# conix-center/pointcloud_stitching

Measured on AMD Instinct MI355X. Metric: Mpoints/s stitched (8x1280x720 streams: deproject+transform+RGB+pack), higher is better.
Workload: dtype f32

## Files before the change

### pointcloud_stitching_amd/csrc/pcs_capi.cpp

```cpp

#include <algorithm>
#include <cmath>
#include <cstdarg>
#include <cstdio>
#include <cstdlib>
#include <cstring>
#include <exception>
#include <new>
#include <string>
#include <vector>

#include "pcs_host.h"

using namespace pcs_host;

namespace pcs_host {

thread_local std::string g_create_err;

int fail(pcs_ctx* c, int status, const char* fmt, ...)
{
    char buf[512];
    va_list ap;
    va_start(ap, fmt);
// ... 946 lines not shown
}

int pcs_process_frames_device_batch(pcs_ctx* c, int n_sets, const uint16_t* const* d_depth, const uint8_t* const* d_color,
                                    int16_t* const* d_payload, size_t payload_shorts, int32_t* const* d_counts)
try {
    if (!c) return PCS_ERR_INVALID_ARG;
    if (n_sets < 0) return fail(c, PCS_ERR_INVALID_ARG, "n_sets %d < 0", n_sets);
    if (n_sets == 0) return PCS_OK;
    if (!d_depth || !d_color || !d_payload) return fail(c, PCS_ERR_INVALID_ARG, "NULL pointer");
    const int S = c->n_streams;
    bool aligned = true;
    for (int k = 0; k < n_sets; k++) {
        if (!d_payload[k]) return fail(c, PCS_ERR_INVALID_ARG, "frame-set %d: NULL payload pointer", k);
        if ((uintptr_t)d_payload[k] & 1u) return fail(c, PCS_ERR_INVALID_ARG, "frame-set %d: payload pointer must be 2-byte aligned", k);
        aligned &= ((uintptr_t)d_payload[k] & 15u) == 0;
        for (int s = 0; s < S; s++) {
            if (!d_depth[(size_t)k * S + s] || !d_color[(size_t)k * S + s])
                return fail(c, PCS_ERR_INVALID_ARG, "frame-set %d stream %d: NULL raster pointer", k, s);
            if ((uintptr_t)d_depth[(size_t)k * S + s] & 1u)
                return fail(c, PCS_ERR_INVALID_ARG, "frame-set %d stream %d: depth pointer not 2-byte aligned", k, s);
        }
    }
    DeviceGuard guard(c->device);
    const int per_launch = std::min(kBatchSets, kBatchEntries / S);
    const bool dense = !has_pred(c->flags) && c->downsample == 1 && c->dense_ok && aligned && per_launch >= 2;
    if (has_pred(c->flags) && c->downsample == 1 && per_launch >= 2 && S <= kLaunchStreams) {
        if (payload_shorts < c->max_payload_points * PCS_POINT_SHORTS)
            return fail(c, PCS_ERR_CAPACITY, "payload buffers hold %zu shorts; with compaction the worst case %zu is required",
                        payload_shorts, c->max_payload_points * PCS_POINT_SHORTS);
        const size_t tt = std::max<uint32_t>(c->total_tiles, 1);
        const size_t row = 2 * tt + (size_t)S + (size_t)(S + 1);
        if (c->batch_scratch_sets < per_launch) {
            if (c->d_batch_scratch) { HIPCHK(c, hipStreamSynchronize(c->stream)); (void)hipFree(c->d_batch_scratch); c->d_batch_scratch = nullptr; }
            c->batch_scratch_sets = 0;
            HIPCHK(c, hipMalloc((void**)&c->d_batch_scratch, sizeof(uint32_t) * row * per_launch));
            c->batch_scratch_sets = per_launch;
        }
        uint32_t* tcounts = c->d_batch_scratch;
        uint32_t* tprefix = tcounts + tt * per_launch;
        uint32_t* kept    = tprefix + tt * per_launch;
        int32_t*  icounts = reinterpret_cast<int32_t*>(kept + (size_t)S * per_launch);
        bool fast = true, ident = true;
        for (int s = 0; s < S; s++) { fast &= c->h_params[s].cert_fast != 0; ident &= c->h_params[s].ident_r != 0; }
        const MathSel sel = !fast ? MathSel::Ieee : (ident ? MathSel::CertIdentR : MathSel::Cert);
        std::pair<hipEvent_t, hipEvent_t> ev{};
        if (c->kernel_timing) {
            int rc = acquire_event_pair(c, ev);
            if (rc) return rc;
            HIPCHK(c, hipEventRecord(ev.first, c->stream));
        }
        for (int k0 = 0; k0 < n_sets; k0 += per_launch) {
            const int nk = std::min(per_launch, n_sets - k0);
            BatchPtrs bp{};
            BatchCounts bc{};
            for (int k = 0; k < nk; k++) {
                bp.payload[k] = reinterpret_cast<uint8_t*>(d_payload[k0 + k]);
                bc.counts[k] = (d_counts && d_counts[k0 + k]) ? d_counts[k0 + k] : icounts + (size_t)k * (S + 1);
                for (int s = 0; s < S; s++) {
                    bp.depth[k * S + s] = d_depth[(size_t)(k0 + k) * S + s];
                    bp.color[k * S + s] = d_color[(size_t)(k0 + k) * S + s];
                }
            }
            HIPCHK(c, launch_compact_batch(c->d_params, S, nk, c->max_points, c->total_tiles, c->flags, sel, bp, bc,
                                           tcounts, tprefix, kept, c->stream));
        }
        if (c->kernel_timing) {
            HIPCHK(c, hipEventRecord(ev.second, c->stream));
            c->ev_pool.push_back(ev);
        }
        return PCS_OK;
    }
    if (!dense) {
        for (int k = 0; k < n_sets; k++) {
            int rc = run_fused_device(c, d_depth + (size_t)k * S, d_color + (size_t)k * S, d_payload[k], payload_shorts,
                                      d_counts ? d_counts[k] : nullptr);
            if (rc) return rc;
        }
        return PCS_OK;
    }
    if (payload_shorts < c->max_payload_points * PCS_POINT_SHORTS)
        return fail(c, PCS_ERR_CAPACITY, "payload buffers hold %zu shorts, %zu needed", payload_shorts,
                    c->max_payload_points * PCS_POINT_SHORTS);
    bool fast = true, ident = true, noovf = true, dd = false, cd = false;
    for (int s = 0; s < S; s++) {
        const StreamParams& q = c->h_params[s];
        fast &= q.cert_fast != 0; ident &= q.ident_r != 0; noovf &= q.no_overflow != 0;
        dd |= q.ddist != 0;
        cd |= q.cdist != 0 || q.tex_half != 0;
    }
    const MathSel sel = !fast ? MathSel::Ieee
                      : noovf ? (ident ? MathSel::CertIdentRNoOvf : MathSel::CertNoOvf)
                              : (ident ? MathSel::CertIdentR : MathSel::Cert);
    std::pair<hipEvent_t, hipEvent_t> ev{};
    if (c->kernel_timing) {
        int rc = acquire_event_pair(c, ev);
        if (rc) return rc;
        HIPCHK(c, hipEventRecord(ev.first, c->stream));
    }
    for (int k0 = 0; k0 < n_sets; k0 += per_launch) {
        const int nk = std::min(per_launch, n_sets - k0);
        BatchPtrs bp{};
        for (int k = 0; k < nk; k++) {
            bp.payload[k] = reinterpret_cast<uint8_t*>(d_payload[k0 + k]);
            for (int s = 0; s < S; s++) {
                bp.depth[k * S + s] = d_depth[(size_t)(k0 + k) * S + s];
                bp.color[k * S + s] = d_color[(size_t)(k0 + k) * S + s];
            }
        }
        HIPCHK(c, launch_fused_dense_batch(c->d_params, S, nk, c->max_points, dd, cd, sel, bp, c->stream));
    }
    if (d_counts)
        for (int k = 0; k < n_sets; k++)
            if (d_counts[k])
                HIPCHK(c, hipMemcpyAsync(d_counts[k], c->d_static_counts, sizeof(int32_t) * (S + 1), hipMemcpyDeviceToDevice, c->stream));
    if (c->kernel_timing) {
        HIPCHK(c, hipEventRecord(ev.second, c->stream));
        c->ev_pool.push_back(ev);
    }
    return PCS_OK;
} catch (const std::exception& ex) {
    return fail(c, PCS_ERR_NOMEM, "pcs_process_frames_device_batch: host allocation failed (%s)", ex.what());
}

int pcs_process_frames(pcs_ctx* c, const uint16_t* const* depth, const uint8_t* const* color, int16_t* stitched,
                       size_t stitched_shorts, int write_header, int* points_per_stream, int* out_size_bytes)
try {
    if (!c) return PCS_ERR_INVALID_ARG;
    if (!depth || !color || !stitched) return fail(c, PCS_ERR_INVALID_ARG, "NULL pointer");
    DeviceGuard guard(c->device);
    int rc;
    for (int s = 0; s < c->n_streams; s++)
        if (!depth[s] || !color[s]) return fail(c, PCS_ERR_INVALID_ARG, "stream %d: NULL raster pointer", s);
    {
        const size_t need = PCS_HEADER_SHORTS + c->max_payload_points * PCS_POINT_SHORTS;
        std::vector<const uint16_t*> zd(c->n_streams);
        std::vector<const uint8_t*> zcol(c->n_streams);
        void* zout = nullptr;
        bool zero_copy = zero_copy_enabled() && stitched_shorts >= need && ((uintptr_t)stitched & 3u) == 0;
        for (int s = 0; s < c->n_streams; s++) {
            void *a = nullptr, *b = nullptr;
            const int va = host_device_view(c, depth[s], (size_t)c->h_params[s].n_points * sizeof(uint16_t), &a);
            const int vb = host_device_view(c, color[s], c->h_params[s].color_bytes, &b);
            if (va < 0 || vb < 0) return partly_locked(c, va < 0 ? "depth raster" : "colour raster", s);
            zero_copy = zero_copy && va == 1 && vb == 1;
            zd[s] = static_cast<const uint16_t*>(a); zcol[s] = static_cast<const uint8_t*>(b);
        }
        {
            const int vo = host_device_view(c, stitched, std::min(stitched_shorts, need) * sizeof(int16_t), &zout);
            if (vo < 0) return partly_locked(c, "stitched buffer", 0);
            zero_copy = zero_copy && vo == 1;
        }
        if (zero_copy) {
            int16_t* zpay = static_cast<int16_t*>(zout) + PCS_HEADER_SHORTS;
            rc = run_fused_device(c, zd.data(), zcol.data(), zpay, c->max_payload_points * PCS_POINT_SHORTS, c->d_counts, true);
            if (rc) return rc;
            std::vector<int32_t> h(c->n_streams + 1);
            HIPCHK(c, hipMemcpyAsync(h.data(), c->d_counts, h.size() * sizeof(int32_t), hipMemcpyDeviceToHost, c->stream));
            HIPCHK(c, hipStreamSynchronize(c->stream));
            const int32_t size = (int32_t)((size_t)h[c->n_streams] * PCS_POINT_BYTES);
            if (write_header) std::memcpy(stitched, &size, sizeof size);
            if (points_per_stream) for (int s = 0; s < c->n_streams; s++) points_per_stream[s] = h[s];
            if (out_size_bytes) *out_size_bytes = size;
            return PCS_OK;
        }
    }
    if ((rc = ensure_rasters(c))) return rc;
    for (int s = 0; s < c->n_streams; s++) {
        const StreamParams& P = c->h_params[s];
        const size_t db = (size_t)P.n_points * sizeof(uint16_t);
        HIPCHK(c, hipMemcpyAsync(c->s_depth[s], depth[s], db, hipMemcpyHostToDevice, c->stream));
        HIPCHK(c, hipMemcpyAsync(c->s_color[s], color[s], P.color_bytes, hipMemcpyHostToDevice, c->stream));
    }
    const size_t max_bytes = c->max_payload_points * PCS_POINT_BYTES;
    if ((rc = ensure(c, c->s_payload, c->s_payload_cap, max_bytes + 16))) return rc;
    rc = run_fused_device(c, c->s_depth.data(), c->s_color.data(), c->s_payload, c->max_payload_points * PCS_POINT_SHORTS,
// ... 436 lines not shown
```

### pointcloud_stitching_amd/csrc/pcs_kernels.hip

```cpp

#include "pcs_kernels_common.h"

#ifndef EMIT_WAVES
#define EMIT_WAVES 6
#endif

namespace pcs {

namespace {

constexpr uint32_t kDenseStageBytes = kTilePoints * PCS_POINT_BYTES;
constexpr uint32_t kStageBytes      = kTilePoints * PCS_POINT_BYTES + 32;

__device__ __forceinline__ void stage_record(uint8_t* lds, uint32_t off, const Record& r)
{
    const bool odd = (off & 2u) != 0u;
    const uint32_t yz = perm(r.zc, r.xy, kHiLo);
    const uint32_t cc = perm(r.b, r.zc, kHiLo);
    const uint32_t h_val = odd ? r.xy : r.b;
    const uint32_t a_val = odd ? yz : r.xy;
    const uint32_t b_val = odd ? cc : r.zc;
    const uint32_t h_off = odd ? off : off + 8u;
    const uint32_t a_off = odd ? off + 2u : off;
    *reinterpret_cast<uint16_t*>(lds + h_off) = (uint16_t)h_val;
// ... 74 lines not shown
__device__ __forceinline__ void dense_tile(const StreamParams& P, const Src& src, const uint8_t* __restrict__ color,
                                           uint32_t tile0, uint32_t n, uint8_t* __restrict__ out_bytes,
                                           uint4* stage)
{
    const uint32_t i0 = tile0 + threadIdx.x * kPointsPerLane;
    PointIn p[8];
    src.load8(P, i0, n, p);

    uint32_t w[20];
    auto fill = [&](auto& cv) {
#pragma unroll
        for (int k = 0; k < 8; k += 2) {
            const Record a = make_record(P, color, p[k], cv);
            const Record b = make_record(P, color, p[k + 1], cv);
            uint32_t* o = w + (k >> 1) * 5;
            o[0] = a.xy;
            o[1] = a.zc;
            o[2] = perm(b.xy, a.b, kLoLo);
            o[3] = perm(b.zc, b.xy, kHiLo);
            o[4] = perm(b.b, b.zc, kHiLo);
        }
    };
    if (Src::Math::kCvtMode == 2) {
        FastCvt<false> fast;
        fill(fast);
        if (__builtin_expect(fast.redo(), 0)) { ExactCvt exact; fill(exact); }
    } else if (Src::Math::kCvtMode == 1) {
        FastCvt<true> fast;
        fill(fast);
        if (__builtin_expect(fast.redo(), 0)) { ExactCvt exact; fill(exact); }
    } else {
        ExactCvt exact;
        fill(exact);
    }
    uint4* mine = stage + threadIdx.x * 5;
#pragma unroll
    for (int k = 0; k < 5; k++) mine[k] = make_uint4(w[4 * k], w[4 * k + 1], w[4 * k + 2], w[4 * k + 3]);
    __syncthreads();

    const uint32_t pts = min(THREADS * kPointsPerLane, n - tile0);
    store_staged<THREADS>(reinterpret_cast<const uint8_t*>(stage), 0u, pts * PCS_POINT_BYTES,
                          out_bytes + (size_t)tile0 * PCS_POINT_BYTES);
}

constexpr uint32_t kWaveStageBytes = 64u * kPointsPerLane * PCS_POINT_BYTES;
constexpr uint32_t kWinPieces      = 3;
constexpr uint32_t kWinBytes       = kWinPieces * 64u * 16u;
constexpr uint32_t kWinZeroWord    = kWaveStageBytes - 16u;
static_assert(kWinBytes + 8u <= kWinZeroWord, "the windows, the dword read past their end and the zero word fit one wave's stage");

template <class T> using cptr = const __attribute__((address_space(4))) T*;

__device__ __forceinline__ void color_stretch(const StreamParams& P, const int32_t (&wp)[3], int32_t crow, int32_t c0, int32_t c1,
                                              uint32_t room, uint32_t& ws, uint32_t& len)
{
    const int32_t lo = min(max((c0 * wp[0] + wp[1]) >> 12, 0), P.cW - 1);
    const int32_t hi = min(max((c1 * wp[0] + wp[2]) >> 12, 0), P.cW - 1);
    const uint32_t row = (uint32_t)crow * (uint32_t)P.stride;
    ws = (row + (uint32_t)lo * (uint32_t)P.bpp) & ~15u;
    const uint32_t we = min((row + (uint32_t)hi * (uint32_t)P.bpp + 4u + 15u) & ~15u, P.color_bytes & ~15u);
    len = min(we > ws ? we - ws : 0u, room);
}

typedef uint32_t u32x4v __attribute__((ext_vector_type(4)));
__device__ __forceinline__ u32x4v load16_asm(const void* base, uint32_t off)
{
    u32x4v v;
    asm volatile("global_load_dwordx4 %0, %1, %2" : "=v"(v) : "v"(off), "s"(base));
    return v;
}
__device__ __forceinline__ uint32_t load4_asm(const void* base, uint32_t off)
{
    uint32_t v;
    asm volatile("global_load_dword %0, %1, %2" : "=v"(v) : "v"(off), "s"(base));
    return v;
}
__device__ __forceinline__ void window_piece(const uint8_t* color, uint32_t off, uint32_t lds)
{
    uint32_t keep;
    asm volatile("s_mov_b32 %0, m0\n\ts_mov_b32 m0, %3\n\ts_nop 0\n\tglobal_load_lds_dwordx4 %1, %2\n\ts_mov_b32 m0, %0"
                 : "=&s"(keep) : "v"(off), "s"(color), "s"(lds) : "memory");
}

template <class Mth, uint32_t THREADS = kBlockThreads>
__device__ __forceinline__ void dense_tile_rowc(const StreamParams& P, const uint16_t* __restrict__ depth,
                                                const uint8_t* __restrict__ color, uint32_t tile0, uint32_t n,
                                                uint8_t* __restrict__ out_bytes, uint4* stage)
{
    static_assert(Mth::kRowConst && Mth::kCvtMode == 2, "the no-overflow row-constant policy");
    const uint32_t i0 = tile0 + threadIdx.x * kPointsPerLane;
    const uint32_t ic = min(i0, n - kPointsPerLane);
    const uint32_t r = P.w_magic ? (__umulhi(ic, P.w_magic) >> P.w_shift) : ic / (uint32_t)P.W;
    const uint32_t c0 = ic - r * (uint32_t)P.W;
    u32x4v dv = load16_asm(depth, ic * 2u);
    u32x4v ma = load16_asm(P.mx, c0 * 4u);
    u32x4v mb = load16_asm(P.mx, c0 * 4u + 16u);
    uint32_t myb = load4_asm(P.my, r * 4u);
    uint32_t crow = load4_asm(P.my, ((uint32_t)P.H + r) * 4u);

    const uint32_t wave = __builtin_amdgcn_readfirstlane(threadIdx.x >> 6);
    const uint32_t iw = tile0 + wave * 64u * kPointsPerLane;
    const uint32_t il = min(iw + 64u * kPointsPerLane, n) - 1u;
    const uint32_t ra = __builtin_amdgcn_readfirstlane(r), rb = __builtin_amdgcn_readlane(r, 63);
    const cptr<int32_t> tab = (cptr<int32_t>)(uintptr_t)(P.my + P.H);
    const int32_t wp[3] = {tab[P.H], tab[P.H + 1], tab[P.H + 2]};
    const uint32_t lrel = wave * kWaveStageBytes;
    uint32_t wsa = 0, lena = 0, wsb = 0, lenb = 0;
    if (iw < n) {
        color_stretch(P, wp, tab[ra], (int32_t)(iw - ra * (uint32_t)P.W), ra == rb ? (int32_t)(il - ra * (uint32_t)P.W) : P.W - 1,
                      kWinBytes, wsa, lena);
        if (rb != ra) color_stretch(P, wp, tab[rb], 0, (int32_t)(il - rb * (uint32_t)P.W), kWinBytes - lena, wsb, lenb);
    }
    const uint32_t lane = threadIdx.x & 63u;
    const uint32_t pieces = max((lena + lenb) >> 4, 1u), pa = lena >> 4;
    const uint32_t lds0 = (uint32_t)(uintptr_t)(__attribute__((address_space(3))) uint8_t*)stage + lrel;
#pragma unroll
    for (uint32_t k = 0; k < kWinPieces; k++) {
        const uint32_t j = min(k * 64u + lane, pieces - 1u);
        window_piece(color, j < pa ? wsa + 16u * j : wsb + 16u * (j - pa), lds0 + k * 1024u);
    }
    if (lane == 0) *reinterpret_cast<uint32_t*>(reinterpret_cast<uint8_t*>(stage) + lrel + kWinZeroWord) = *(cptr<uint32_t>)(uintptr_t)color;

    static_assert(kWinPieces == 3, "the wait below leaves the window's requests in flight");
    asm volatile("s_waitcnt vmcnt(3)" : "+v"(dv), "+v"(ma), "+v"(mb), "+v"(myb), "+v"(crow));
    PointIn p[8];
    {
        const uint32_t dw[4] = {dv.x, dv.y, dv.z, dv.w};
        const uint32_t mxs[8] = {ma.x, ma.y, ma.z, ma.w, mb.x, mb.y, mb.z, mb.w};
#pragma unroll
        for (int k = 0; k < 8; k++) {
            const uint32_t d = (k & 1) ? (dw[k >> 1] >> 16) : (dw[k >> 1] & 0xFFFFu);
            p[k] = deproject_pixel_rowc<Mth>(P, d, __uint_as_float(mxs[k]), __uint_as_float(myb), (int)crow);
        }
    }
    FastCvt<false> cv;
    uint32_t xy[8], zz[8], ci[8];
#pragma unroll
    for (int k = 0; k < 8; k++) {
        const float ax = world_mm(P.M + 0, p[k].X, p[k].Y, p[k].Z);
        const float ay = world_mm(P.M + 4, p[k].X, p[k].Y, p[k].Z);
        const float az = world_mm(P.M + 8, p[k].X, p[k].Y, p[k].Z);
        xy[k] = perm((uint32_t)cv.cvt(ay), (uint32_t)cv.cvt(ax), kLoLo);
        zz[k] = (uint32_t)cv.cvt(az);
        const int32_t xi = cv.pixel(__fmaf_rn(p[k].u, P.c_w_f, 0.5f), P.cW - 1, P.c_wm1_f);
        ci[k] = __umul24((uint32_t)xi, (uint32_t)P.bpp) + __umul24((uint32_t)__float_as_int(p[k].v), (uint32_t)P.stride);
    }
    const bool in_a = r == ra;
    const uint32_t ws = in_a ? wsa : wsb, len = in_a ? lena : lenb;
    const uint32_t wn = len > 3u ? len - 3u : 0u;
    const uint32_t lb = lrel + (in_a ? 0u : lena), lz = lrel + kWinZeroWord;
    asm volatile("s_waitcnt vmcnt(0)" : "+v"(ci[0]), "+v"(ci[1]), "+v"(ci[2]), "+v"(ci[3]), "+v"(ci[4]), "+v"(ci[5]), "+v"(ci[6]),
                 "+v"(ci[7]) :: "memory");
    uint32_t wc[8];
    bool miss = false;
#pragma unroll
    for (int k = 0; k < 8; k++) {
        const uint32_t o = ci[k] - ws;
        const bool in = o < wn;
        const uint32_t* qa = reinterpret_cast<const uint32_t*>(reinterpret_cast<const uint8_t*>(stage) + (in ? (lb + o) & ~3u : lz));
        wc[k] = __builtin_amdgcn_alignbyte(qa[1], qa[0], ci[k]);
        miss |= !in && ci[k] != 0u;
    }
    if (__builtin_expect(miss, 0)) {
#pragma unroll
        for (int k = 0; k < 8; k++) {
            if (!(ci[k] - ws < wn) && ci[k] != 0u) {
                ExactCvt exact;
                uint32_t shift;
                const uint32_t off = exact.window(ci[k], P.color_bytes - 4u, shift);
                uint32_t g;
                __builtin_memcpy(&g, color + off, 4);
                wc[k] = g >> shift;
            }
        }
    }
    uint32_t w[20];
#pragma unroll
    for (int k = 0; k < 8; k += 2) {
        const Record a{xy[k], perm(wc[k], zz[k], kLoLo), __builtin_amdgcn_ubfe(wc[k], 16, 8)};
        const Record b{xy[k + 1], perm(wc[k + 1], zz[k + 1], kLoLo), __builtin_amdgcn_ubfe(wc[k + 1], 16, 8)};
        uint32_t* o = w + (k >> 1) * 5;
        o[0] = a.xy;
        o[1] = a.zc;
        o[2] = perm(b.xy, a.b, kLoLo);
        o[3] = perm(b.zc, b.xy, kHiLo);
        o[4] = perm(b.b, b.zc, kHiLo);
    }
    uint4* mine = stage + threadIdx.x * 5;
#pragma unroll
    for (int k = 0; k < 5; k++) mine[k] = make_uint4(w[4 * k], w[4 * k + 1], w[4 * k + 2], w[4 * k + 3]);
    __syncthreads();

    const uint32_t pts = min(THREADS * kPointsPerLane, n - tile0);
    store_staged<THREADS>(reinterpret_cast<const uint8_t*>(stage), 0u, pts * PCS_POINT_BYTES,
                          out_bytes + (size_t)tile0 * PCS_POINT_BYTES);
}

template <class Src, bool PRED, bool DS1>
__device__ __forceinline__ void generic_tile(const StreamParams& P, const Src& src, const uint8_t* __restrict__ color,
                                             uint32_t tile0, uint32_t n, uint32_t flags, uint32_t ds,
                                             uint32_t g0, uint32_t out_first, uint8_t* __restrict__ payload_bytes,
                                             uint8_t* stage, uint32_t* wsum)
{
    if (DS1) ds = 1u;
    const uint32_t i0 = tile0 + threadIdx.x * kPointsPerLane;
    PointIn p[8];
    src.load8(P, i0, n, p);

    uint32_t keep, ex = 0;
    if (PRED) {
        keep = keep_mask8(p, i0, n, flags);
        uint32_t wave_total;
        ex = wave_exclusive_scan(__popc(keep), wave_total);
        if ((threadIdx.x & 63) == 63) wsum[threadIdx.x >> 6] = wave_total;
    } else {
        const uint32_t mine = (i0 < n) ? min(8u, n - i0) : 0u;
        keep = (1u << mine) - 1u;
    }

    Record rec[8];
    auto fill = [&](auto& cv) {
#pragma unroll
        for (int k = 0; k < 8; k++) rec[k] = make_record(P, color, p[k], cv);
    };
    if (Src::Math::kCvtMode == 2) {
        FastCvt<false> fast;
        fill(fast);
        if (__builtin_expect(fast.redo(), 0)) { ExactCvt exact; fill(exact); }
// ... 137 lines not shown
        if (__builtin_expect(fast.redo(), 0)) { ExactCvt exact; fill(exact); }
    } else if (Mth::kCvtMode == 1) {
        FastCvt<true> fast;
        fill(fast);
        if (__builtin_expect(fast.redo(), 0)) { ExactCvt exact; fill(exact); }
    } else {
        ExactCvt exact;
        fill(exact);
    }

    uint32_t own = 0, tot = 0;
    const uint32_t first = gtile - t;
    for (uint32_t j = first + threadIdx.x; j < gtile; j += kBlockThreads) own += desc_wait(a.desc + j, a.gen, a.error);
    if ((int)threadIdx.x < s) tot = desc_wait(a.stream_desc + stream0 + threadIdx.x, a.gen, a.error);
    const uint32_t tot_lane = tot;
    own = wave_sum(own);
    tot = wave_sum(tot);
    if (lane == 0) { psum[wave] = own; psum[4 + wave] = tot; }
    __syncthreads();
    const uint32_t own_excl = psum[0] + psum[1] + psum[2] + psum[3];
    const uint32_t chain = a.chain_in ? *a.chain_in : 0u;
    const uint32_t q_lo = chain + psum[4] + psum[5] + psum[6] + psum[7] + own_excl;
    if (threadIdx.x == 0 && t == tiles_s - 1) {
        __hip_atomic_store(a.stream_desc + stream0 + s, desc_pack(a.gen, kDescReady, own_excl + tile_kept), __ATOMIC_RELAXED,
                           __HIP_MEMORY_SCOPE_AGENT);
        a.stream_end[stream0 + s] = q_lo + tile_kept;
    }
    if (a.counts && s == n_launch - 1 && t == tiles_s - 1) {
        if ((int)threadIdx.x < s) a.counts[stream0 + threadIdx.x] = (int32_t)tot_lane;
        if (threadIdx.x == 0) {
            a.counts[stream0 + s] = (int32_t)(own_excl + tile_kept);
            if (a.last_launch) a.counts[a.n_total] = (int32_t)(q_lo + tile_kept);
        }
    }

    uint8_t* gdst = payload_bytes + (size_t)q_lo * PCS_POINT_BYTES;
    const uint32_t head = (uint32_t)((uintptr_t)gdst & 15u);
    uint32_t rank = lane_first;
#pragma unroll
    for (int k = 0; k < 8; k++) {
        if ((keep >> k) & 1u) {
            stage_record(stage, head + rank * PCS_POINT_BYTES, rec[k]);
            rank++;
        }
    }
    __syncthreads();
    store_staged(stage, head, tile_kept * PCS_POINT_BYTES, gdst);
}



template <bool DDIST, bool CDIST, class Mth, uint32_t THREADS = kBlockThreads>
__global__ __launch_bounds__(THREADS, 7)
void pcs_fused_dense_kernel(const StreamParams* __restrict__ params, int stream0, FramePtrs fp,
                            uint8_t* __restrict__ payload_bytes)
{
    __shared__ uint4 stage[THREADS * kPointsPerLane * PCS_POINT_BYTES / 16];
    const int s = blockIdx.y;
    const StreamParams& P = params[stream0 + s];
    request_constants(P, fp.depth[s], fp.color[s], payload_bytes);
    const uint32_t n = P.n_points;
    const uint32_t tile0 = blockIdx.x * (THREADS * kPointsPerLane);
    if (tile0 >= n) return;
    if constexpr (Mth::kRowConst) {
        dense_tile_rowc<Mth, THREADS>(P, fp.depth[s], fp.color[s], tile0, n, payload_bytes + (size_t)P.out_base * PCS_POINT_BYTES, stage);
    } else {
        DepthSource<DDIST, CDIST, Mth> src{fp.depth[s]};
        dense_tile<DepthSource<DDIST, CDIST, Mth>, THREADS>(P, src, fp.color[s], tile0, n, payload_bytes + (size_t)P.out_base * PCS_POINT_BYTES, stage);
    }
}

template <bool DDIST, bool CDIST, class Mth>
__global__ __launch_bounds__(kBlockThreads, 7)
void pcs_fused_dense_batch_kernel(const StreamParams* __restrict__ params, BatchPtrs bp)
{
    __shared__ uint4 stage[kDenseStageBytes / 16];
    const int s = blockIdx.y;
    const StreamParams& P = params[s];
    const int e = blockIdx.z * gridDim.y + s;
    request_constants(P, bp.depth[e], bp.color[e], bp.payload[blockIdx.z]);
    const uint32_t n = P.n_points;
    const uint32_t tile0 = blockIdx.x * kTilePoints;
    if (tile0 >= n) return;
    DepthSource<DDIST, CDIST, Mth> src{bp.depth[e]};
    dense_tile(P, src, bp.color[e], tile0, n, bp.payload[blockIdx.z] + (size_t)P.out_base * PCS_POINT_BYTES, stage);
}

constexpr int kCountTiles = 2;
template <bool DDIST, bool CDIST>
__device__ __forceinline__ void count_tiles(const StreamParams& P, const uint16_t* __restrict__ dp, uint32_t flags,
                                            uint32_t* __restrict__ tile_counts, uint32_t (*wsum)[4])
{
    const uint32_t n = P.n_points;
    const uint32_t tile_first = blockIdx.x * kCountTiles;
    if (tile_first * kTilePoints >= n) return;
    uint32_t c[kCountTiles];
    const bool cut = (flags & PCS_FLAG_CUTOFF) != 0;
    if (P.z_zero_iff_d_zero && (!cut || P.cut_dmax != 0u)) {
        const uint32_t dmax = cut ? P.cut_dmax : 0xFFFFu;
        uint4 dv[kCountTiles];
        const bool aligned = ((uintptr_t)dp & 15) == 0 && n >= 8;
        if (aligned) {
#pragma unroll
            for (int q = 0; q < kCountTiles; q++) {
                const uint32_t i0 = (tile_first + q) * kTilePoints + threadIdx.x * kPointsPerLane;
                dv[q] = *reinterpret_cast<const uint4*>(dp + ((i0 + 8 <= n) ? i0 : 0u));
            }
        } else {
#pragma unroll
            for (int q = 0; q < kCountTiles; q++) dv[q] = make_uint4(0, 0, 0, 0);
        }
#pragma unroll
        for (int q = 0; q < kCountTiles; q++) {
            const uint32_t i0 = (tile_first + q) * kTilePoints + threadIdx.x * kPointsPerLane;
            uint32_t dw[4] = {dv[q].x, dv[q].y, dv[q].z, dv[q].w};
            if (!(aligned && i0 + 8 <= n)) {
                dw[0] = dw[1] = dw[2] = dw[3] = 0u;
                for (uint32_t k = 0; k < 8 && i0 + k < n; k++) dw[k >> 1] |= (uint32_t)dp[i0 + k] << ((k & 1u) * 16u);
            }
            uint32_t rng = 0, nz = 0;
#pragma unroll
            for (int k = 0; k < 8; k++) {
                const uint32_t d = (k & 1) ? (dw[k >> 1] >> 16) : (dw[k >> 1] & 0xFFFFu);
                nz  |= (uint32_t)(d != 0u) << k;
                rng |= (uint32_t)(d != 0u && d <= dmax) << k;
            }
            c[q] = __popc(keep_from_bits(rng, nz, i0, n, flags));
        }
    } else {
        DepthSource<DDIST, CDIST> src{dp};
#pragma unroll
        for (int q = 0; q < kCountTiles; q++) {
            const uint32_t i0 = (tile_first + q) * kTilePoints + threadIdx.x * kPointsPerLane;
            PointIn p[8];
            src.load8(P, i0, n, p);
            c[q] = __popc(keep_mask8(p, i0, n, flags));
        }
    }
#pragma unroll
    for (int q = 0; q < kCountTiles; q++) {
        const uint32_t w = wave_sum(c[q]);
        if ((threadIdx.x & 63) == 0) wsum[q][threadIdx.x >> 6] = w;
    }
    __syncthreads();
    if (threadIdx.x < kCountTiles && (tile_first + threadIdx.x) * kTilePoints < n)
        tile_counts[P.tile_base + tile_first + threadIdx.x] =
            wsum[threadIdx.x][0] + wsum[threadIdx.x][1] + wsum[threadIdx.x][2] + wsum[threadIdx.x][3];
}

template <bool DDIST, bool CDIST>
__global__ __launch_bounds__(kBlockThreads)
void pcs_fused_count_kernel(const StreamParams* __restrict__ params, int stream0, FramePtrs fp, uint32_t flags,
                            uint32_t* __restrict__ tile_counts)
{
    __shared__ uint32_t wsum[kCountTiles][4];
    const int s = blockIdx.y;
    count_tiles<DDIST, CDIST>(params[stream0 + s], fp.depth[s], flags, tile_counts, wsum);
}

template <bool DDIST, bool CDIST>
__global__ __launch_bounds__(kBlockThreads)
void pcs_fused_count_batch_kernel(const StreamParams* __restrict__ params, BatchPtrs bp, uint32_t flags,
                                  uint32_t* __restrict__ tile_counts, uint32_t total_tiles)
{
    __shared__ uint32_t wsum[kCountTiles][4];
    const int s = blockIdx.y;
    count_tiles<DDIST, CDIST>(params[s], bp.depth[blockIdx.z * gridDim.y + s], flags,
                              tile_counts + (size_t)blockIdx.z * total_tiles, wsum);
// ... 449 lines not shown
    if (math != MathSel::Ieee && !any_ddist) {
        const bool ident = (math == MathSel::CertIdentR || math == MathSel::CertIdentRNoOvf);
        const bool noovf = (math == MathSel::CertNoOvf || math == MathSel::CertIdentRNoOvf) && !any_cdist;
        if (noovf)      { if (ident) L(false, false, CertIdentNoOvf); else L(false, false, CertNoOvf); }
        else if (ident) { if (any_cdist) L(false, true, CertMath<true>); else L(false, false, CertMath<true>); }
        else            { if (any_cdist) L(false, true, CertMath<false>); else L(false, false, CertMath<false>); }
    } else {
        if (any_ddist) { if (any_cdist) L(true, true, IeeeMath); else L(true, false, IeeeMath); }
        else           { if (any_cdist) L(false, true, IeeeMath); else L(false, false, IeeeMath); }
    }
#undef L
    return hipGetLastError();
}

hipError_t launch_fused_count(const StreamParams* d_params, int stream0, int n_launch, uint32_t max_points,
                              uint32_t flags, const FramePtrs& fp, uint32_t* d_tile_counts, hipStream_t st)
{
    if (n_launch <= 0 || max_points == 0) return hipSuccess;
    const uint32_t tiles = (max_points + kTilePoints - 1) / kTilePoints;
    const dim3 grid((tiles + kCountTiles - 1) / kCountTiles, (unsigned)n_launch, 1);
    hipLaunchKernelGGL((pcs_fused_count_kernel<true, false>), grid, dim3(kBlockThreads), 0, st,
                       d_params, stream0, fp, flags, d_tile_counts);
    return hipGetLastError();
}

hipError_t launch_scan(const StreamParams* d_params, int n_streams, int downsample,
                       const uint32_t* d_tile_counts, uint32_t* d_tile_prefix, uint32_t* d_stream_kept,
                       int32_t* d_counts, uint32_t* d_arrive, hipStream_t st)
{
    hipLaunchKernelGGL(pcs_scan_kernel, dim3((unsigned)n_streams), dim3(1024), 0, st, d_params, 0, n_streams, 0u,
                       (uint32_t)downsample, d_tile_counts, d_tile_prefix, d_stream_kept, d_counts, d_arrive);
    return hipGetLastError();
}

hipError_t launch_fused_emit(const StreamParams* d_params, int stream0, int n_launch, uint32_t max_points,
                             uint32_t flags, int downsample, MathSel math, const FramePtrs& fp,
                             const uint32_t* d_tile_prefix, const uint32_t* d_stream_kept,
                             int16_t* d_payload, int32_t* d_total_out, int n_total_streams, hipStream_t st)
{
    if (n_launch <= 0 || max_points == 0) return hipSuccess;
    const dim3 grid = tile_grid(max_points, n_launch);
    const bool pred = (flags & (PCS_FLAG_CUTOFF | PCS_FLAG_DROP_INVALID)) != 0;
    const bool ds1 = downsample == 1;
    uint8_t* out = reinterpret_cast<uint8_t*>(d_payload);
#define L(PR, D1, M) hipLaunchKernelGGL((pcs_fused_emit_kernel<PR, D1, M>), grid, dim3(kBlockThreads), 0, st, d_params, \
                                        stream0, fp, flags, (uint32_t)downsample, d_tile_prefix, d_stream_kept, out, \
                                        d_total_out, n_total_streams)
#define LM(M) do { if (pred) { if (ds1) L(true, true, M); else L(true, false, M); } \
                   else      { if (ds1) L(false, true, M); else L(false, false, M); } } while (0)
    const bool ident = (math == MathSel::CertIdentR || math == MathSel::CertIdentRNoOvf);
    if (math == MathSel::Ieee) LM(IeeeMath); else if (ident) LM(CertMath<true>); else LM(CertMath<false>);
#undef LM
#undef L
    return hipGetLastError();
}

hipError_t launch_fused_compact(const StreamParams* d_params, int stream0, int n_launch, uint32_t launch_tiles,
                                MathSel math, const FramePtrs& fp, const CompactLaunch& cl, int16_t* d_payload,
                                hipStream_t st)
{
    if (n_launch <= 0 || launch_tiles == 0) return hipSuccess;
    CompactArgs a;
    a.ticket = cl.d_ticket; a.ticket_base = cl.ticket_base; a.desc = cl.d_desc; a.stream_desc = cl.d_stream_desc;
    a.stream_end = cl.d_stream_end;
    a.chain_in = cl.d_chain_in; a.error = cl.d_error; a.gen = cl.gen & 0x3FFFFFFFu; a.flags = cl.flags;
    a.counts = cl.d_counts; a.n_total = cl.n_total; a.last_launch = cl.last_launch;
    uint8_t* out = reinterpret_cast<uint8_t*>(d_payload);
    if (math != MathSel::Ieee)
        hipLaunchKernelGGL((pcs_fused_compact_kernel<CertMath<false>>), dim3(launch_tiles), dim3(kBlockThreads), 0, st,
                           d_params, stream0, n_launch, fp, a, out);
    else
        hipLaunchKernelGGL((pcs_fused_compact_kernel<IeeeMath>), dim3(launch_tiles), dim3(kBlockThreads), 0, st,
                           d_params, stream0, n_launch, fp, a, out);
    return hipGetLastError();
}

hipError_t launch_fused_dense_batch(const StreamParams* d_params, int n_streams, int n_sets, uint32_t max_points,
                                    bool any_ddist, bool any_cdist, MathSel math, const BatchPtrs& bp, hipStream_t st)
{
    if (n_streams <= 0 || n_sets <= 0 || max_points == 0) return hipSuccess;
    if (n_streams * n_sets > kBatchEntries || n_sets > kBatchSets) return hipErrorInvalidValue;
    const dim3 grid((max_points + kTilePoints - 1) / kTilePoints, (unsigned)n_streams, (unsigned)n_sets);
#define L(DD, CD, M) hipLaunchKernelGGL((pcs_fused_dense_batch_kernel<DD, CD, M>), grid, dim3(kBlockThreads), 0, st, d_params, bp)
    if (math != MathSel::Ieee && !any_ddist) {
        const bool ident = (math == MathSel::CertIdentR || math == MathSel::CertIdentRNoOvf);
        const bool noovf = (math == MathSel::CertNoOvf || math == MathSel::CertIdentRNoOvf) && !any_cdist;
        if (noovf)      { if (ident) L(false, false, CertIdentNoOvf); else L(false, false, CertNoOvf); }
        else if (ident) { if (any_cdist) L(false, true, CertMath<true>); else L(false, false, CertMath<true>); }
        else            { if (any_cdist) L(false, true, CertMath<false>); else L(false, false, CertMath<false>); }
    } else {
        if (any_ddist) { if (any_cdist) L(true, true, IeeeMath); else L(true, false, IeeeMath); }
        else           { if (any_cdist) L(false, true, IeeeMath); else L(false, false, IeeeMath); }
    }
#undef L
    return hipGetLastError();
}

hipError_t launch_compact_batch(const StreamParams* d_params, int n_streams, int n_sets, uint32_t max_points,
                                uint32_t total_tiles, uint32_t flags, MathSel math, const BatchPtrs& bp,
                                const BatchCounts& bc, uint32_t* d_tile_counts, uint32_t* d_tile_prefix,
                                uint32_t* d_stream_kept, hipStream_t st)
{
    if (n_streams <= 0 || n_sets <= 0 || max_points == 0) return hipSuccess;
    if (n_streams * n_sets > kBatchEntries || n_sets > kBatchSets) return hipErrorInvalidValue;
    const uint32_t tiles = (max_points + kTilePoints - 1) / kTilePoints;
    hipLaunchKernelGGL((pcs_fused_count_batch_kernel<true, false>),
                       dim3((tiles + kCountTiles - 1) / kCountTiles, (unsigned)n_streams, (unsigned)n_sets),
                       dim3(kBlockThreads), 0, st, d_params, bp, flags, d_tile_counts, total_tiles);
    hipLaunchKernelGGL(pcs_scan_batch_kernel, dim3((unsigned)n_streams, (unsigned)n_sets), dim3(1024), 0, st, d_params,
                       d_tile_counts, d_tile_prefix, d_stream_kept, total_tiles, bc);
    const dim3 grid(tiles, (unsigned)n_streams, (unsigned)n_sets);
#define L(M) hipLaunchKernelGGL((pcs_fused_emit_batch_kernel<M>), grid, dim3(kBlockThreads), 0, st, d_params, bp, flags, \
                                d_tile_prefix, d_stream_kept, total_tiles, bc)
    const bool ident = (math == MathSel::CertIdentR || math == MathSel::CertIdentRNoOvf);
    if (math == MathSel::Ieee) L(IeeeMath); else if (ident) L(CertMath<true>); else L(CertMath<false>);
#undef L
    return hipGetLastError();
}

hipError_t launch_pack_batch(const StreamParams* d_params, const PackBatch& pb, int n, uint32_t max_points, bool aligned,
                             hipStream_t st)
{
    if (n <= 0 || max_points == 0) return hipSuccess;
    if (n > kPackBatch) return hipErrorInvalidValue;
    const dim3 grid = tile_grid(max_points, n);
    if (aligned) hipLaunchKernelGGL((pcs_pack_batch_kernel<true>), grid, dim3(kBlockThreads), 0, st, d_params, pb);
    else         hipLaunchKernelGGL((pcs_pack_batch_kernel<false>), grid, dim3(kBlockThreads), 0, st, d_params, pb);
    return hipGetLastError();
}

hipError_t launch_certify_color_row(const StreamParams* d_params, int stream, int rows, int32_t* d_crow, unsigned long long* d_bad, hipStream_t st)
{
    if (rows <= 0) return hipSuccess;
    hipLaunchKernelGGL(pcs_certify_color_row_kernel, dim3((unsigned)rows), dim3(256), 0, st, d_params, stream, d_crow, d_bad);
    return hipGetLastError();
}

hipError_t launch_verify_div_const(float c, float rc, int32_t dim, unsigned long long* d_bad, hipStream_t st)
{
    hipLaunchKernelGGL(pcs_verify_div_const_kernel, dim3(8192), dim3(256), 0, st, c, rc, dim, d_bad);
    return hipGetLastError();
}

hipError_t launch_pack_dense(const StreamParams* d_params, int stream, const VertexPtrs& vp,
                             int16_t* d_out, hipStream_t st)
{
    if (vp.n_points == 0) return hipSuccess;
    if (small_launch(vp.n_points, 1))
        hipLaunchKernelGGL((pcs_pack_dense_kernel<kSmallThreads>), dim3((vp.n_points + kSmallTilePoints - 1) / kSmallTilePoints),
                           dim3(kSmallThreads), 0, st, d_params, stream, vp, reinterpret_cast<uint8_t*>(d_out));
    else
        hipLaunchKernelGGL((pcs_pack_dense_kernel<kBlockThreads>), tile_grid(vp.n_points, 1), dim3(kBlockThreads), 0, st,
                           d_params, stream, vp, reinterpret_cast<uint8_t*>(d_out));
    return hipGetLastError();
}

hipError_t launch_pack_count(const StreamParams* d_params, int stream, const VertexPtrs& vp, uint32_t flags,
                             uint32_t* d_tile_counts, hipStream_t st)
{
    if (vp.n_points == 0) return hipSuccess;
    hipLaunchKernelGGL(pcs_pack_count_kernel, tile_grid(vp.n_points, 1), dim3(kBlockThreads), 0, st,
                       d_params, stream, vp, flags, d_tile_counts);
    return hipGetLastError();
}

hipError_t launch_pack_scan(uint32_t n_tiles, const uint32_t* d_tile_counts, uint32_t* d_tile_prefix,
// ... 58 lines not shown
```

Before: 338,400.

## Route dense batch through row-constant window kernel for identity-rotation streams

Adds a host-side check that picks a new row-constant no-overflow math path when every stream has an ident_r==2 extrinsic, width divisible by 8 and 16-byte color alignment. The batched dense kernel then dispatches to dense_tile_rowc, which uses a simplified deprojection that skips the v division (color row is constant per image row) and a color window staged into LDS. Transform matrix and scalars are pinned in SGPRs to avoid reloads. The gain depends on the test cameras meeting these conditions; otherwise it falls back to the existing path.

```diff
diff --git a/pointcloud_stitching_amd/csrc/pcs_capi.cpp b/pointcloud_stitching_amd/csrc/pcs_capi.cpp
--- a/pointcloud_stitching_amd/csrc/pcs_capi.cpp
+++ b/pointcloud_stitching_amd/csrc/pcs_capi.cpp
@@ -1052,15 +1052,18 @@
         return fail(c, PCS_ERR_CAPACITY, "payload buffers hold %zu shorts, %zu needed", payload_shorts,
                     c->max_payload_points * PCS_POINT_SHORTS);
     bool fast = true, ident = true, noovf = true, dd = false, cd = false;
+    bool rowc = true;
     for (int s = 0; s < S; s++) {
         const StreamParams& q = c->h_params[s];
         fast &= q.cert_fast != 0; ident &= q.ident_r != 0; noovf &= q.no_overflow != 0;
+        rowc &= q.ident_r == 2 && (q.W & 7) == 0 && q.color_bytes >= 16;
         dd |= q.ddist != 0;
         cd |= q.cdist != 0 || q.tex_half != 0;
     }
-    const MathSel sel = !fast ? MathSel::Ieee
-                      : noovf ? (ident ? MathSel::CertIdentRNoOvf : MathSel::CertNoOvf)
-                              : (ident ? MathSel::CertIdentR : MathSel::Cert);
+    MathSel sel = !fast ? MathSel::Ieee
+                : noovf ? (ident ? MathSel::CertIdentRNoOvf : MathSel::CertNoOvf)
+                        : (ident ? MathSel::CertIdentR : MathSel::Cert);
+    if (sel == MathSel::CertIdentRNoOvf && rowc) sel = MathSel::CertRowConstNoOvf;
     std::pair<hipEvent_t, hipEvent_t> ev{};
     if (c->kernel_timing) {
         int rc = acquire_event_pair(c, ev);
diff --git a/pointcloud_stitching_amd/csrc/pcs_kernels.hip b/pointcloud_stitching_amd/csrc/pcs_kernels.hip
--- a/pointcloud_stitching_amd/csrc/pcs_kernels.hip
+++ b/pointcloud_stitching_amd/csrc/pcs_kernels.hip
@@ -180,6 +180,24 @@
                  : "=&s"(keep) : "v"(off), "s"(color), "s"(lds) : "memory");
 }
 
+template <class Mth>
+__device__ __forceinline__ PointIn deproject_pixel_win(const StreamParams& P, uint32_t d, float mx, float my)
+{
+    const float z = __fmul_rn(P.depth_scale, (float)d);
+    PointIn p;
+    p.X = __fmul_rn(z, mx);
+    p.Y = __fmul_rn(z, my);
+    p.Z = z;
+    const float P0 = __fadd_rn(p.X, P.t[0]);
+    const float P2 = p.Z;
+    float x, y_unused;
+    Mth::div2(P0, P0, P2, x, y_unused);
+    const float px = __fadd_rn(__fmul_rn(x, P.c_fx), P.c_ppx);
+    p.u = Mth::div_const(px, P.c_w_f, P.c_rw);
+    p.v = 0.0f;
+    return p;
+}
+
 template <class Mth, uint32_t THREADS = kBlockThreads>
 __device__ __forceinline__ void dense_tile_rowc(const StreamParams& P, const uint16_t* __restrict__ depth,
                                                 const uint8_t* __restrict__ color, uint32_t tile0, uint32_t n,
@@ -218,7 +236,13 @@
         window_piece(color, j < pa ? wsa + 16u * j : wsb + 16u * (j - pa), lds0 + k * 1024u);
     }
     if (lane == 0) *reinterpret_cast<uint32_t*>(reinterpret_cast<uint8_t*>(stage) + lrel + kWinZeroWord) = *(cptr<uint32_t>)(uintptr_t)color;
-
+    float M[12];
+#pragma unroll
+    for (int k = 0; k < 12; k++) M[k] = P.M[k];
+    float c_wm1_f = P.c_wm1_f;
+    uint32_t bpp = (uint32_t)P.bpp, stride = (uint32_t)P.stride;
+    asm volatile("" : "+s"(M[0]), "+s"(M[1]), "+s"(M[2]), "+s"(M[3]), "+s"(M[4]), "+s"(M[5]), "+s"(M[6]), "+s"(M[7]), "+s"(M[8]),
+                      "+s"(M[9]), "+s"(M[10]), "+s"(M[11]), "+s"(c_wm1_f), "+s"(bpp), "+s"(stride));
     static_assert(kWinPieces == 3, "the wait below leaves the window's requests in flight");
     asm volatile("s_waitcnt vmcnt(3)" : "+v"(dv), "+v"(ma), "+v"(mb), "+v"(myb), "+v"(crow));
     PointIn p[8];
@@ -228,20 +252,21 @@
 #pragma unroll
         for (int k = 0; k < 8; k++) {
             const uint32_t d = (k & 1) ? (dw[k >> 1] >> 16) : (dw[k >> 1] & 0xFFFFu);
-            p[k] = deproject_pixel_rowc<Mth>(P, d, __uint_as_float(mxs[k]), __uint_as_float(myb), (int)crow);
+            p[k] = deproject_pixel_win<Mth>(P, d, __uint_as_float(mxs[k]), __uint_as_float(myb));
         }
     }
     FastCvt<false> cv;
     uint32_t xy[8], zz[8], ci[8];
+    const uint32_t row_off = __umul24(crow, stride);
 #pragma unroll
     for (int k = 0; k < 8; k++) {
-        const float ax = world_mm(P.M + 0, p[k].X, p[k].Y, p[k].Z);
-        const float ay = world_mm(P.M + 4, p[k].X, p[k].Y, p[k].Z);
-        const float az = world_mm(P.M + 8, p[k].X, p[k].Y, p[k].Z);
+        const float ax = world_mm(M + 0, p[k].X, p[k].Y, p[k].Z);
+        const float ay = world_mm(M + 4, p[k].X, p[k].Y, p[k].Z);
+        const float az = world_mm(M + 8, p[k].X, p[k].Y, p[k].Z);
         xy[k] = perm((uint32_t)cv.cvt(ay), (uint32_t)cv.cvt(ax), kLoLo);
         zz[k] = (uint32_t)cv.cvt(az);
-        const int32_t xi = cv.pixel(__fmaf_rn(p[k].u, P.c_w_f, 0.5f), P.cW - 1, P.c_wm1_f);
-        ci[k] = __umul24((uint32_t)xi, (uint32_t)P.bpp) + __umul24((uint32_t)__float_as_int(p[k].v), (uint32_t)P.stride);
+        const int32_t xi = cv.pixel(__fmaf_rn(p[k].u, P.c_w_f, 0.5f), P.cW - 1, c_wm1_f);
+        ci[k] = p[k].Z != 0.0f ? __umul24((uint32_t)xi, bpp) + row_off : 0u;
     }
     const bool in_a = r == ra;
     const uint32_t ws = in_a ? wsa : wsb, len = in_a ? lena : lenb;
@@ -545,8 +570,12 @@
     const uint32_t n = P.n_points;
     const uint32_t tile0 = blockIdx.x * kTilePoints;
     if (tile0 >= n) return;
-    DepthSource<DDIST, CDIST, Mth> src{bp.depth[e]};
-    dense_tile(P, src, bp.color[e], tile0, n, bp.payload[blockIdx.z] + (size_t)P.out_base * PCS_POINT_BYTES, stage);
+    if constexpr (Mth::kRowConst) {
+        dense_tile_rowc<Mth>(P, bp.depth[e], bp.color[e], tile0, n, bp.payload[blockIdx.z] + (size_t)P.out_base * PCS_POINT_BYTES, stage);
+    } else {
+        DepthSource<DDIST, CDIST, Mth> src{bp.depth[e]};
+        dense_tile(P, src, bp.color[e], tile0, n, bp.payload[blockIdx.z] + (size_t)P.out_base * PCS_POINT_BYTES, stage);
+    }
 }
 
 constexpr int kCountTiles = 2;
@@ -1162,6 +1191,12 @@
     if (n_streams * n_sets > kBatchEntries || n_sets > kBatchSets) return hipErrorInvalidValue;
     const dim3 grid((max_points + kTilePoints - 1) / kTilePoints, (unsigned)n_streams, (unsigned)n_sets);
 #define L(DD, CD, M) hipLaunchKernelGGL((pcs_fused_dense_batch_kernel<DD, CD, M>), grid, dim3(kBlockThreads), 0, st, d_params, bp)
+    if (math == MathSel::CertRowConstNoOvf) {
+        bool aligned = !any_ddist && !any_cdist;
+        for (int k = 0; k < n_streams * n_sets; k++) aligned &= ((((uintptr_t)bp.color[k]) | ((uintptr_t)bp.depth[k])) & 15u) == 0;
+        if (aligned) { L(false, false, CertRowConstNoOvf); return hipGetLastError(); }
+        math = MathSel::CertIdentRNoOvf;
+    }
     if (math != MathSel::Ieee && !any_ddist) {
         const bool ident = (math == MathSel::CertIdentR || math == MathSel::CertIdentRNoOvf);
         const bool noovf = (math == MathSel::CertNoOvf || math == MathSel::CertIdentRNoOvf) && !any_cdist;
```

After: 342,300 (median of 6 runs). +1.2%, better.
